# houzhijian/CONE

Measured on AMD Instinct MI355X. Metric: windows/sec + queries/sec, Ego4D-NLQ win_len=90 d=256 top-k=20, higher is better.
Workload: dtype f32

## Files before the change

### cone_amd/csrc/attention.hip

```cpp
#include "common.h"

#ifndef CONE_ATTN_NT
#define CONE_ATTN_NT 0
#endif

namespace cone {

constexpr float kQScale = 0.17677669529663687f;
constexpr float kQScaleLog2 = 0.17677669529663687f * 1.4426950408889634f;


typedef float f32x4m __attribute__((ext_vector_type(4)));
typedef float f32x2m __attribute__((ext_vector_type(2)));

__device__ __forceinline__ float lane_xor(float v, int lane, int mask) {
    return __int_as_float(__builtin_amdgcn_ds_bpermute((lane ^ mask) << 2, __float_as_int(v)));
}

template <int NKT>
__device__ __forceinline__ float attn_softmax(f32x4m (&sc)[NKT], int L, int lane, int lg) {
    const int lim = L - lg;
    float m = -INFINITY;
#pragma unroll
    for (int kt = 0; kt < NKT; ++kt) {
        if (16 * (kt + 1) > L) {
#pragma unroll
            for (int r = 0; r < 4; ++r) sc[kt][r] = (16 * kt + 4 * r < lim) ? sc[kt][r] : -INFINITY;
        }
#pragma unroll
        for (int r = 0; r < 4; ++r) m = fmaxf(m, sc[kt][r]);
    }
    m = fmaxf(m, lane_xor(m, lane, 16));
    m = fmaxf(m, lane_xor(m, lane, 32));
    const f32x2m m2 = {m, m};
    f32x2m l2 = {0.f, 0.f};
#pragma unroll
    for (int kt = 0; kt < NKT; ++kt) {
        f32x2m a = sc[kt].xy - m2, b = sc[kt].zw - m2;
        a.x = __builtin_amdgcn_exp2f(a.x); a.y = __builtin_amdgcn_exp2f(a.y);
        b.x = __builtin_amdgcn_exp2f(b.x); b.y = __builtin_amdgcn_exp2f(b.y);
        sc[kt].xy = a; sc[kt].zw = b;
        l2 += a;
        l2 += b;
    }
    float l = l2.x + l2.y;
    l += lane_xor(l, lane, 16);
    l += lane_xor(l, lane, 32);
    return 1.0f / l;
}

__device__ __forceinline__ void attn_normalise(f32x4m& o0, f32x4m& o1, float inv, int lane, int lg) {
#pragma unroll
    for (int r = 0; r < 4; ++r) {
        const float s = __int_as_float(__builtin_amdgcn_ds_bpermute(((lane & 48) + 4 * lg + r) << 2, __float_as_int(inv)));
        o0[r] *= s;
        o1[r] *= s;
    }
}

template <int NKT, int MODE_>
__global__ __launch_bounds__(64 * NKT, (NKT > 12 ? 4 : 6)) void enc_attn16_kernel(AttnSrc a, float* __restrict__ OUT,
                                                                 const int* __restrict__ off) {
    constexpr int MODE = MODE_ & 3;
    constexpr bool TXT = (MODE_ & 4) != 0;
    constexpr int KP = 16 * NKT, LDK = KP + 2, LDV = 36, NT = 64 * NKT;
    constexpr bool DYN = NKT > 12;
    __shared__ float KsT_s[DYN ? 4 : 32 * LDK];
    __shared__ __attribute__((aligned(16))) float Vs_s[DYN ? 4 : KP * LDV];
    extern __shared__ __attribute__((aligned(16))) float attn_dyn[];
    float* const KsT = DYN ? attn_dyn : KsT_s;
    float* const Vs = DYN ? attn_dyn + 32 * LDK : Vs_s;
    const int b = blockIdx.y, head = blockIdx.x;
    const int t0 = off[b];
    const int L = off[b + 1] - t0;
    if (L <= 0) return;
    const int tid = threadIdx.x, lane = tid & 63;
    const int wave = __builtin_amdgcn_readfirstlane(tid >> 6);
    const int li = lane & 15, lg = lane >> 4;
    const unsigned hc = head * 32;
    int lv = 0;
    const float *qb = nullptr, *kb = nullptr, *vb = nullptr, *tb = nullptr, *pb = nullptr;
    unsigned sq = 768, sk = 768, sv = 768;
    int pbase = 0;
    if (MODE != ATTN_PACKED) {
        lv = a.vlen[b];
        pbase = lv * (lv - 1) / 2;
        pb = a.pos_qk + hc;
    }
    if (MODE == ATTN_GATHER) {
        qb = a.qkv_vid + (size_t)a.vrow0[b] * 768 + hc;
        tb = a.qkv_txt + ((ptrdiff_t)a.trow0[b] - lv) * 768 + hc;
    } else {
        sq = a.ldq; sk = a.ldk; sv = a.ldv;
        qb = a.Q + (size_t)t0 * sq + hc; kb = a.K + (size_t)t0 * sk + hc; vb = a.V + (size_t)t0 * sv + hc;
    }
    const int zrow = a.pos_zero_row;
    const float* tpb = nullptr;
    if (TXT) tpb = a.txt_pos_qk + ((ptrdiff_t)a.trow0[b] - lv) * 512 + hc;
    auto prow = [&](int row) -> const float* {
        if (TXT && row >= lv) return tpb + (unsigned)row * 512u;
        return pb + (unsigned)(row < lv ? pbase + row : zrow) * 512u;
    };

    const int q0 = wave * 16;
    const int kr = tid >> 3;
    const unsigned c4 = (tid & 7) * 4;
    f32x4m qx[2], qt[2], kv[2], vv[2], kt_[2];
    {
        const int qrow = min(q0 + li, L - 1);
        const float* qp;
        if (MODE == ATTN_GATHER) qp = (qrow < lv ? qb : tb) + (unsigned)qrow * 768u + 8u * lg;
        else qp = qb + (unsigned)qrow * sq + 8u * lg;
        qx[0] = *reinterpret_cast<const f32x4m*>(qp);
        qx[1] = *reinterpret_cast<const f32x4m*>(qp + 4);
        if (MODE != ATTN_PACKED) {
            const float* pr = prow(qrow) + 8u * lg;
            qt[0] = *reinterpret_cast<const f32x4m*>(pr);
            qt[1] = *reinterpret_cast<const f32x4m*>(pr + 4);
        }
    }
#pragma unroll
    for (int it = 0; it < 2; ++it) {
        const int row = min(kr + it * (NT / 8), L - 1);
        if (MODE == ATTN_GATHER) {
            const float* rp = (row < lv ? qb : tb) + (unsigned)row * 768u + c4;
            kv[it] = *reinterpret_cast<const f32x4m*>(rp + 256);
            vv[it] = *reinterpret_cast<const f32x4m*>(rp + 512);
        } else {
#if CONE_ATTN_NT
            kv[it] = __builtin_nontemporal_load(reinterpret_cast<const f32x4m*>(kb + (unsigned)row * sk + c4));
            vv[it] = __builtin_nontemporal_load(reinterpret_cast<const f32x4m*>(vb + (unsigned)row * sv + c4));
#else
            kv[it] = *reinterpret_cast<const f32x4m*>(kb + (unsigned)row * sk + c4);
            vv[it] = *reinterpret_cast<const f32x4m*>(vb + (unsigned)row * sv + c4);
#endif
        }
        if (MODE != ATTN_PACKED)
            kt_[it] = *reinterpret_cast<const f32x4m*>(prow(row) + 256u + c4);
    }
    float qv[8];
    {
        f32x4m x0 = qx[0], x1 = qx[1];
        if (MODE != ATTN_PACKED) { x0 += qt[0]; x1 += qt[1]; }
        x0 *= kQScaleLog2; x1 *= kQScaleLog2;
#pragma unroll
        for (int j = 0; j < 4; ++j) { qv[j] = x0[j]; qv[4 + j] = x1[j]; }
    }
#pragma unroll
    for (int it = 0; it < 2; ++it) {
        const int key = kr + it * (NT / 8);
        f32x4m k4 = kv[it];
        if (MODE != ATTN_PACKED) k4 += kt_[it];
        const int pos = (key & ~15) + 4 * (key & 3) + ((key >> 2) & 3);
        float* kd = KsT + c4 * LDK + pos;
        kd[0] = k4[0]; kd[LDK] = k4[1]; kd[2 * LDK] = k4[2]; kd[3 * LDK] = k4[3];
        *reinterpret_cast<f32x4m*>(Vs + pos * LDV + c4) = vv[it];
    }
    __syncthreads();
    if (q0 >= L) return;

    f32x4m sc[NKT];
#pragma unroll
    for (int kt = 0; kt < NKT; ++kt) sc[kt] = f32x4m{0.f, 0.f, 0.f, 0.f};
#pragma unroll
    for (int st = 0; st < 8; ++st) {
        const float* kp = KsT + (8 * lg + st) * LDK + li;
#pragma unroll
        for (int kt = 0; kt < NKT; ++kt)
            sc[kt] = __builtin_amdgcn_mfma_f32_16x16x4f32(kp[kt * 16], qv[st], sc[kt], 0, 0, 0);
    }
    const float inv = attn_softmax<NKT>(sc, L, lane, lg);
    f32x4m o0 = {0.f, 0.f, 0.f, 0.f}, o1 = o0;
#pragma unroll
    for (int kt = 0; kt < NKT; ++kt) {
        const float* vp = Vs + (kt * 16 + 4 * lg) * LDV + li;
#pragma unroll
        for (int r = 0; r < 4; ++r) {
            if (kt < NKT - 2 || 16 * kt + 4 * r < L) {
                o0 = __builtin_amdgcn_mfma_f32_16x16x4f32(sc[kt][r], vp[r * LDV], o0, 0, 0, 0);
                o1 = __builtin_amdgcn_mfma_f32_16x16x4f32(sc[kt][r], vp[r * LDV + 16], o1, 0, 0, 0);
            }
        }
    }
    attn_normalise(o0, o1, inv, lane, lg);
    float* ob = OUT + (size_t)t0 * 256 + hc;
    const int qr0 = q0 + 4 * lg;
    const unsigned oo = (unsigned)qr0 * 256u + li;
#pragma unroll
    for (int r = 0; r < 4; ++r) {
        if (qr0 + r < L) {
            ob[oo + 256u * r] = o0[r];
            ob[oo + 256u * r + 16u] = o1[r];
        }
    }
}

template <int NKT, int MODE>
__global__ __launch_bounds__(256, 2) void enc_attn_wave_kernel(AttnSrc a, float* __restrict__ OUT,
                                                               const int* __restrict__ off) {
    const int b = blockIdx.y;
    const int lane = threadIdx.x & 63;
    const int head = blockIdx.x * 4 + __builtin_amdgcn_readfirstlane(threadIdx.x >> 6);
    const int t0 = off[b];
    const int L = off[b + 1] - t0;
    if (L <= 0) return;
    const int li = lane & 15, lg = lane >> 4;
    const unsigned hc = head * 32;
    int lv = 0, pbase = 0;
    const float *qb = nullptr, *kb = nullptr, *vb = nullptr, *tb = nullptr, *pb = nullptr;
    unsigned sq = 768, sk = 768, sv = 768;
    if (MODE != ATTN_PACKED) { lv = a.vlen[b]; pbase = lv * (lv - 1) / 2; pb = a.pos_qk + hc; }
    if (MODE == ATTN_GATHER) {
        qb = a.qkv_vid + (size_t)a.vrow0[b] * 768 + hc;
        tb = a.qkv_txt + ((ptrdiff_t)a.trow0[b] - lv) * 768 + hc;
    } else {
        sq = a.ldq; sk = a.ldk; sv = a.ldv;
        qb = a.Q + (size_t)t0 * sq + hc; kb = a.K + (size_t)t0 * sk + hc; vb = a.V + (size_t)t0 * sv + hc;
    }
    const int zrow = a.pos_zero_row;
    auto qptr = [&](int tok) { return MODE == ATTN_GATHER ? (tok < lv ? qb : tb) + (unsigned)tok * 768u : qb + (unsigned)tok * sq; };
    auto kptr = [&](int tok) { return MODE == ATTN_GATHER ? (tok < lv ? qb : tb) + (unsigned)tok * 768u + 256 : kb + (unsigned)tok * sk; };
    auto vptr = [&](int tok) { return MODE == ATTN_GATHER ? (tok < lv ? qb : tb) + (unsigned)tok * 768u + 512 : vb + (unsigned)tok * sv; };
    auto pptr = [&](int tok) { return pb + (unsigned)(tok < lv ? pbase + tok : zrow) * 512u; };
    f32x4m qx[2], qt[2];
    auto load_q = [&](int q0) {
        const int qrow = min(q0 + li, L - 1);
        const float* qp = qptr(qrow) + 8 * lg;
        qx[0] = *reinterpret_cast<const f32x4m*>(qp);
        qx[1] = *reinterpret_cast<const f32x4m*>(qp + 4);
        if (MODE != ATTN_PACKED) {
            const float* ap = pptr(qrow) + 8 * lg;
            qt[0] = *reinterpret_cast<const f32x4m*>(ap);
            qt[1] = *reinterpret_cast<const f32x4m*>(ap + 4);
        }
    };
    load_q(0);
    float kreg[NKT][8];
#pragma unroll
    for (int kt = 0; kt < NKT; ++kt) {
        const int key = min(16 * kt + 4 * (li & 3) + (li >> 2), L - 1);
        const float* kp_ = kptr(key) + 8 * lg;
#pragma unroll
        for (int u = 0; u < 2; ++u) {
            f32x4m k4 = *reinterpret_cast<const f32x4m*>(kp_ + 4 * u);
            if (MODE != ATTN_PACKED) k4 += *reinterpret_cast<const f32x4m*>(pptr(key) + 256 + 8 * lg + 4 * u);
#pragma unroll
            for (int j = 0; j < 4; ++j) kreg[kt][4 * u + j] = k4[j];
        }
    }
    float vreg[NKT][4][2];
#pragma unroll
    for (int kt = 0; kt < NKT; ++kt)
#pragma unroll
        for (int r = 0; r < 4; ++r) {
            const float* vp_ = vptr(min(16 * kt + 4 * r + lg, L - 1));
            vreg[kt][r][0] = vp_[li];
            vreg[kt][r][1] = vp_[16 + li];
        }
    for (int q0 = 0; q0 < L; q0 += 16) {
        float qv[8];
        {
            f32x4m x0 = qx[0], x1 = qx[1];
            if (MODE != ATTN_PACKED) { x0 += qt[0]; x1 += qt[1]; }
            x0 *= kQScaleLog2; x1 *= kQScaleLog2;
#pragma unroll
            for (int j = 0; j < 4; ++j) { qv[j] = x0[j]; qv[4 + j] = x1[j]; }
        }
        load_q(q0 + 16 < L ? q0 + 16 : q0);
        f32x4m sc[NKT];
#pragma unroll
        for (int kt = 0; kt < NKT; ++kt) sc[kt] = f32x4m{0.f, 0.f, 0.f, 0.f};
#pragma unroll
        for (int st = 0; st < 8; ++st)
#pragma unroll
            for (int kt = 0; kt < NKT; ++kt)
                sc[kt] = __builtin_amdgcn_mfma_f32_16x16x4f32(kreg[kt][st], qv[st], sc[kt], 0, 0, 0);
        const float inv = attn_softmax<NKT>(sc, L, lane, lg);
        f32x4m o0 = {0.f, 0.f, 0.f, 0.f}, o1 = o0;
#pragma unroll
        for (int kt = 0; kt < NKT; ++kt)
#pragma unroll
            for (int r = 0; r < 4; ++r) {
                o0 = __builtin_amdgcn_mfma_f32_16x16x4f32(sc[kt][r], vreg[kt][r][0], o0, 0, 0, 0);
                o1 = __builtin_amdgcn_mfma_f32_16x16x4f32(sc[kt][r], vreg[kt][r][1], o1, 0, 0, 0);
            }
        attn_normalise(o0, o1, inv, lane, lg);
#pragma unroll
        for (int r = 0; r < 4; ++r) {
            const int qrow = q0 + 4 * lg + r;
            if (qrow < L) {
                float* dst = OUT + (size_t)(t0 + qrow) * 256 + hc + li;
                dst[0] = o0[r];
                dst[16] = o1[r];
            }
        }
    }
}

template <int MODE>
static int launch_enc_attn_t(const AttnSrc& a, float* OUT, const int* off, int B, int Lmax, hipStream_t s) {
    const int nkt = max(6, (Lmax + 15) / 16);
    if (a.form == 2 && nkt <= 9 && !(MODE & 4)) {
        dim3 wgrid(2, B);
#define CONE_ATTNW(N) case N: hipLaunchKernelGGL((enc_attn_wave_kernel<N, (MODE & 3)>), wgrid, dim3(256), 0, s, a, OUT, off); break;
        switch (nkt) { CONE_ATTNW(6) CONE_ATTNW(7) CONE_ATTNW(8) CONE_ATTNW(9) }
#undef CONE_ATTNW
        CONE_LAUNCH_CHECK();
        return 0;
    }
    dim3 grid(8, B);
#define CONE_ATTN16(N) case N: hipLaunchKernelGGL((enc_attn16_kernel<N, MODE>), grid, dim3(64 * N), 0, s, a, OUT, off); break;
#define CONE_ATTN16D(N)                                                                                                     \
    case N: {                                                                                                               \
        constexpr int bytes = (32 * (16 * N + 2) + 16 * N * 36) * 4;                                                        \
        static DeviceOnce once;                                                                                             \
        CONE_CHECK_HIP(device_once(once, [] {                                                                               \
            return hipFuncSetAttribute((const void*)enc_attn16_kernel<N, MODE>, hipFuncAttributeMaxDynamicSharedMemorySize, bytes); \
        }));                                                                                                                \
        hipLaunchKernelGGL((enc_attn16_kernel<N, MODE>), grid, dim3(64 * N), bytes, s, a, OUT, off);                        \
        break;                                                                                                              \
    }
    switch (nkt) {
        CONE_ATTN16(6)
        CONE_ATTN16(7) CONE_ATTN16(8) CONE_ATTN16(9) CONE_ATTN16(10) CONE_ATTN16(11) CONE_ATTN16(12)
        CONE_ATTN16D(13) CONE_ATTN16D(14) CONE_ATTN16D(15) CONE_ATTN16D(16)
    }
#undef CONE_ATTN16
#undef CONE_ATTN16D
    CONE_LAUNCH_CHECK();
    return 0;
}

int launch_enc_attn(int mode, const AttnSrc& a, float* OUT, const int* off, int B, int Lmax, hipStream_t s) {
    CONE_REQUIRE(Lmax >= 1 && Lmax <= 256, "enc attention: window length %d not in [1,256]", Lmax);
    if (B <= 0) return 0;
    ProfScope ps(PK_ENC_ATTN, B, Lmax, mode, nullptr, s);
    switch (mode) {
        case ATTN_PACKED:
            CONE_REQUIRE(a.Q && a.K && a.V, "enc attention: packed mode needs Q, K, V");
            return launch_enc_attn_t<ATTN_PACKED>(a, OUT, off, B, Lmax, s);
        case ATTN_GATHER:
            CONE_REQUIRE(a.qkv_vid && a.qkv_txt && a.pos_qk && a.vrow0 && a.vlen && a.trow0 && a.pos_zero_row >= 0,
                         "enc attention: gather mode needs the layer-0 caches");
            if (a.txt_pos_qk) return launch_enc_attn_t<ATTN_GATHER | 4>(a, OUT, off, B, Lmax, s);
            return launch_enc_attn_t<ATTN_GATHER>(a, OUT, off, B, Lmax, s);
        case ATTN_POSADD:
            CONE_REQUIRE(a.Q && a.K && a.V && a.pos_qk && a.vlen && a.pos_zero_row >= 0,
                         "enc attention: pos-add mode needs Q, K, V, pos_qk, vlen");
            if (a.txt_pos_qk) {
                CONE_REQUIRE(a.trow0, "enc attention: text position rows need trow0");
                return launch_enc_attn_t<ATTN_POSADD | 4>(a, OUT, off, B, Lmax, s);
            }
            return launch_enc_attn_t<ATTN_POSADD>(a, OUT, off, B, Lmax, s);
    }
    set_error("enc attention: unknown mode %d", mode);
    return CONE_E_INVALID;
}

constexpr int kSmallMaxKeys = 192;
template <int MQ>
__global__ __launch_bounds__(64) void small_attn_kernel(const float* __restrict__ Q, int ldq,
                                                        const float* __restrict__ K, int ldk,
                                                        const float* __restrict__ V, int ldv,
                                                        float* __restrict__ OUT, int ldo,
                                                        const int* __restrict__ off, int nq) {
    __shared__ float qs[MQ][32];
    __shared__ float ps[MQ][kSmallMaxKeys];
    const int b = blockIdx.x, head = blockIdx.y, lane = threadIdx.x;
    const int k0 = off ? off[b] : b * nq;
    const int L = off ? off[b + 1] - k0 : nq;
    for (int i = lane; i < nq * 8; i += 64) {
        const int qi = i >> 3, c = i & 7;
        const float4 x = *reinterpret_cast<const float4*>(Q + (size_t)(b * nq + qi) * ldq + head * 32 + c * 4);
        qs[qi][c * 4] = x.x * kQScale; qs[qi][c * 4 + 1] = x.y * kQScale;
        qs[qi][c * 4 + 2] = x.z * kQScale; qs[qi][c * 4 + 3] = x.w * kQScale;
    }
    __syncthreads();
    float sc[3][MQ];
#pragma unroll
    for (int jj = 0; jj < 3; ++jj) {
        const int j = lane + 64 * jj;
#pragma unroll
        for (int qi = 0; qi < MQ; ++qi) sc[jj][qi] = -INFINITY;
        if (j < L) {
            float kv[32];
            const float* kp = K + (size_t)(k0 + j) * ldk + head * 32;
#pragma unroll
            for (int u = 0; u < 8; ++u) {
                const float4 x = reinterpret_cast<const float4*>(kp)[u];
                kv[4 * u] = x.x; kv[4 * u + 1] = x.y; kv[4 * u + 2] = x.z; kv[4 * u + 3] = x.w;
            }
#pragma unroll
            for (int qi = 0; qi < MQ; ++qi)
                if (qi < nq) {
                    float a = 0.f;
#pragma unroll
                    for (int d = 0; d < 32; ++d) a = fmaf(qs[qi][d], kv[d], a);
                    sc[jj][qi] = a;
                }
        }
    }
#pragma unroll
    for (int qi = 0; qi < MQ; ++qi)
        if (qi < nq) {
            const float m = wave_max(fmaxf(fmaxf(sc[0][qi], sc[1][qi]), sc[2][qi]));
            float e[3], l = 0.f;
#pragma unroll
            for (int jj = 0; jj < 3; ++jj) {
                e[jj] = (lane + 64 * jj < L) ? expf(sc[jj][qi] - m) : 0.f;
                l += e[jj];
            }
            const float inv = 1.0f / wave_sum(l);
#pragma unroll
            for (int jj = 0; jj < 3; ++jj)
                if (lane + 64 * jj < L) ps[qi][lane + 64 * jj] = e[jj] * inv;
        }
    __syncthreads();
    const int d = lane & 31, h = lane >> 5;
    float o[MQ];
#pragma unroll
    for (int qi = 0; qi < MQ; ++qi) o[qi] = 0.f;
    for (int j = h; j < L; j += 2) {
        const float v = V[(size_t)(k0 + j) * ldv + head * 32 + d];
#pragma unroll
        for (int qi = 0; qi < MQ; ++qi)
            if (qi < nq) o[qi] = fmaf(ps[qi][j], v, o[qi]);
    }
#pragma unroll
    for (int qi = 0; qi < MQ; ++qi)
        if (qi < nq) {
            const float t = o[qi] + __shfl_xor(o[qi], 32, 64);
            if (h == 0) OUT[(size_t)(b * nq + qi) * ldo + head * 32 + d] = t;
        }
}

template <int NQ>
__global__ __launch_bounds__(256) void dec_self_attn_kernel(const float* __restrict__ Q, int ldq, const float* __restrict__ K,
                                                            int ldk, const float* __restrict__ V, int ldv,
                                                            float* __restrict__ OUT, int ldo, int B) {
    const int b = blockIdx.x * 4 + (threadIdx.x >> 6);
    if (b >= B) return;
    const int lane = threadIdx.x & 63;
    float4 q[NQ], k[NQ], v[NQ];
#pragma unroll
    for (int i = 0; i < NQ; ++i) {
        const size_t row = (size_t)b * NQ + i;
        q[i] = reinterpret_cast<const float4*>(Q + row * ldq)[lane];
        k[i] = reinterpret_cast<const float4*>(K + row * ldk)[lane];
        v[i] = reinterpret_cast<const float4*>(V + row * ldv)[lane];
    }
#pragma unroll
    for (int i = 0; i < NQ; ++i) {
        float sc[NQ];
        float m = -INFINITY;
#pragma unroll
        for (int j = 0; j < NQ; ++j) {
            float d = ((q[i].x * kQScale) * k[j].x + (q[i].y * kQScale) * k[j].y) + ((q[i].z * kQScale) * k[j].z + (q[i].w * kQScale) * k[j].w);
            d += __shfl_xor(d, 1, 64);
            d += __shfl_xor(d, 2, 64);
            d += __shfl_xor(d, 4, 64);
            sc[j] = d;
            m = fmaxf(m, d);
        }
        float l = 0.f;
#pragma unroll
        for (int j = 0; j < NQ; ++j) { sc[j] = expf(sc[j] - m); l += sc[j]; }
        const float inv = 1.0f / l;
        float4 o = make_float4(0.f, 0.f, 0.f, 0.f);
#pragma unroll
        for (int j = 0; j < NQ; ++j) {
            const float p = sc[j] * inv;
            o.x = fmaf(p, v[j].x, o.x); o.y = fmaf(p, v[j].y, o.y); o.z = fmaf(p, v[j].z, o.z); o.w = fmaf(p, v[j].w, o.w);
        }
        reinterpret_cast<float4*>(OUT + ((size_t)b * NQ + i) * ldo)[lane] = o;
    }
}

int launch_small_attn(const float* Q, int ldq, const float* K, int ldk, const float* V, int ldv, float* OUT,
                      int ldo, const int* off, int B, int nq, int Lmax, hipStream_t s) {
    CONE_REQUIRE(nq >= 1 && nq <= 16, "decoder attention: num_queries=%d not in [1,16]", nq);
    CONE_REQUIRE(Lmax <= kSmallMaxKeys, "decoder attention: %d keys > %d", Lmax, kSmallMaxKeys);
    if (B <= 0) return 0;
    if (!off && (ldq | ldk | ldv | ldo) % 4 == 0) {
#define CONE_DSA(N)                                                                                                            \
        if (nq == N) {                                                                                                         \
            hipLaunchKernelGGL(dec_self_attn_kernel<N>, dim3((B + 3) / 4), dim3(256), 0, s, Q, ldq, K, ldk, V, ldv, OUT, ldo, B); \
            CONE_LAUNCH_CHECK();                                                                                               \
            return 0;                                                                                                          \
        }
        CONE_DSA(5) CONE_DSA(3) CONE_DSA(8) CONE_DSA(10)
#undef CONE_DSA
    }
    if (nq <= 8)
        hipLaunchKernelGGL(small_attn_kernel<8>, dim3(B, 8), dim3(64), 0, s, Q, ldq, K, ldk, V, ldv, OUT, ldo, off, nq);
    else
        hipLaunchKernelGGL(small_attn_kernel<16>, dim3(B, 8), dim3(64), 0, s, Q, ldq, K, ldk, V, ldv, OUT, ldo, off, nq);
    CONE_LAUNCH_CHECK();
    return 0;
}

}
```

Before: 379,500.

## Split encoder attention into full and short-window paths, byte-offset addressing

Adds separate compile-time paths for windows that fill the last two key tiles and for shorter windows. The short path skips QK and PV matrix-core work on the two trailing key tiles and avoids exponentials on fully masked tiles. It also rewrites global addressing to precomputed byte offsets, stores unguarded output rows when a wave's 16 queries are all valid, and adds asm barriers to shape instruction scheduling in the exp/sum loop. The cost is code duplication and higher register pressure, and a new stride cap is checked at launch.

Result: no change. 383,100 (median of 6 runs) (+0.9%).

```diff
diff --git a/cone_amd/csrc/attention.hip b/cone_amd/csrc/attention.hip
--- a/cone_amd/csrc/attention.hip
+++ b/cone_amd/csrc/attention.hip
@@ -17,31 +17,78 @@
     return __int_as_float(__builtin_amdgcn_ds_bpermute((lane ^ mask) << 2, __float_as_int(v)));
 }
 
-template <int NKT>
-__device__ __forceinline__ float attn_softmax(f32x4m (&sc)[NKT], int L, int lane, int lg) {
+#ifndef CONE_ATTN_PK
+#define CONE_ATTN_PK 0
+#endif
+template <bool FIRST>
+__device__ __forceinline__ void attn_exp_tile(f32x4m& s, float m, f32x2m& l2) {
+#if CONE_ATTN_PK
+    const f32x2m m2 = {m, m};
+    f32x2m a = s.xy - m2, b = s.zw - m2;
+    asm("" : "+v"(a));
+    asm("" : "+v"(b));
+    a.x = __builtin_amdgcn_exp2f(a.x); a.y = __builtin_amdgcn_exp2f(a.y);
+    b.x = __builtin_amdgcn_exp2f(b.x); b.y = __builtin_amdgcn_exp2f(b.y);
+    asm("" : "+v"(a));
+    asm("" : "+v"(b));
+    s.xy = a; s.zw = b;
+    if (FIRST) l2 = a; else l2 += a;
+    l2 += b;
+    asm("" : "+v"(l2));
+#else
+    float e[4];
+#pragma unroll
+    for (int r = 0; r < 4; ++r) {
+        e[r] = s[r] - m;
+        asm("" : "+v"(e[r]));
+        e[r] = __builtin_amdgcn_exp2f(e[r]);
+        s[r] = e[r];
+    }
+    float lx = l2.x, ly = l2.y;
+    if (FIRST) { lx = e[0]; ly = e[1]; }
+    else {
+        lx += e[0];
+        asm("" : "+v"(lx));
+        ly += e[1];
+        asm("" : "+v"(ly));
+    }
+    lx += e[2];
+    asm("" : "+v"(lx));
+    ly += e[3];
+    asm("" : "+v"(ly));
+    l2.x = lx; l2.y = ly;
+#endif
+}
+
+__device__ __forceinline__ void attn_mask_tile(f32x4m& s, int kt, int lim) {
+#pragma unroll
+    for (int r = 0; r < 4; ++r) s[r] = (16 * kt + 4 * r < lim) ? s[r] : -INFINITY;
+}
+
+template <int NKT, bool FULL>
+__device__ __forceinline__ float attn_softmax_path(f32x4m (&sc)[NKT], int L, int lane, int lg) {
     const int lim = L - lg;
+    if (!FULL) __builtin_assume(L <= 16 * (NKT - 2));
     float m = -INFINITY;
 #pragma unroll
     for (int kt = 0; kt < NKT; ++kt) {
-        if (16 * (kt + 1) > L) {
-#pragma unroll
-            for (int r = 0; r < 4; ++r) sc[kt][r] = (16 * kt + 4 * r < lim) ? sc[kt][r] : -INFINITY;
+        if (FULL) {
+            if (kt == NKT - 1 || (kt == NKT - 2 && 16 * (kt + 1) > L)) attn_mask_tile(sc[kt], kt, lim);
+        } else {
+            if (16 * kt >= L) continue;
+            if (16 * (kt + 1) > L) attn_mask_tile(sc[kt], kt, lim);
         }
 #pragma unroll
         for (int r = 0; r < 4; ++r) m = fmaxf(m, sc[kt][r]);
     }
     m = fmaxf(m, lane_xor(m, lane, 16));
     m = fmaxf(m, lane_xor(m, lane, 32));
-    const f32x2m m2 = {m, m};
     f32x2m l2 = {0.f, 0.f};
-#pragma unroll
-    for (int kt = 0; kt < NKT; ++kt) {
-        f32x2m a = sc[kt].xy - m2, b = sc[kt].zw - m2;
-        a.x = __builtin_amdgcn_exp2f(a.x); a.y = __builtin_amdgcn_exp2f(a.y);
-        b.x = __builtin_amdgcn_exp2f(b.x); b.y = __builtin_amdgcn_exp2f(b.y);
-        sc[kt].xy = a; sc[kt].zw = b;
-        l2 += a;
-        l2 += b;
+    attn_exp_tile<true>(sc[0], m, l2);
+#pragma unroll
+    for (int kt = 1; kt < NKT; ++kt) {
+        if (!FULL && 16 * kt >= L) sc[kt] = f32x4m{0.f, 0.f, 0.f, 0.f};
+        else attn_exp_tile<false>(sc[kt], m, l2);
     }
     float l = l2.x + l2.y;
     l += lane_xor(l, lane, 16);
@@ -49,6 +96,12 @@
     return 1.0f / l;
 }
 
+template <int NKT>
+__device__ __forceinline__ float attn_softmax(f32x4m (&sc)[NKT], int L, int lane, int lg) {
+    if (L > 16 * (NKT - 2)) return attn_softmax_path<NKT, true>(sc, L, lane, lg);
+    return attn_softmax_path<NKT, false>(sc, L, lane, lg);
+}
+
 __device__ __forceinline__ void attn_normalise(f32x4m& o0, f32x4m& o1, float inv, int lane, int lg) {
 #pragma unroll
     for (int r = 0; r < 4; ++r) {
@@ -56,6 +109,55 @@
         o0[r] *= s;
         o1[r] *= s;
     }
+}
+
+__device__ __forceinline__ f32x4m ldg4(const float* base, unsigned byte_off) {
+    return *reinterpret_cast<const f32x4m*>(reinterpret_cast<const char*>(base) + byte_off);
+}
+__device__ __forceinline__ void stg(float* base, unsigned byte_off, float v) {
+    *reinterpret_cast<float*>(reinterpret_cast<char*>(base) + byte_off) = v;
+}
+
+template <int NKT, bool FULL>
+__device__ __forceinline__ float attn_core16(const float* KsT, const float* Vs, const float (&qv)[8], int L, int lane, int li,
+                                             int lg, f32x4m& o0, f32x4m& o1) {
+    constexpr int LDK = 16 * NKT + 2, LDV = 36;
+    f32x4m sc[NKT];
+#pragma unroll
+    for (int kt = 0; kt < NKT; ++kt) sc[kt] = f32x4m{0.f, 0.f, 0.f, 0.f};
+    if (FULL) {
+#pragma unroll
+        for (int st = 0; st < 8; ++st) {
+            const float* kp = KsT + (8 * lg + st) * LDK + li;
+#pragma unroll
+            for (int kt = 0; kt < NKT; ++kt)
+                sc[kt] = __builtin_amdgcn_mfma_f32_16x16x4f32(kp[kt * 16], qv[st], sc[kt], 0, 0, 0);
+        }
+    } else {
+#pragma unroll
+        for (int kt = 0; kt < NKT - 2; ++kt) {
+            if (16 * kt < L) {
+#pragma unroll
+                for (int st = 0; st < 8; ++st)
+                    sc[kt] = __builtin_amdgcn_mfma_f32_16x16x4f32(KsT[(8 * lg + st) * LDK + li + kt * 16], qv[st], sc[kt], 0, 0, 0);
+            }
+        }
+    }
+    const float inv = attn_softmax_path<NKT, FULL>(sc, L, lane, lg);
+    o0 = f32x4m{0.f, 0.f, 0.f, 0.f};
+    o1 = o0;
+#pragma unroll
+    for (int kt = 0; kt < (FULL ? NKT : NKT - 2); ++kt) {
+        const float* vp = Vs + (kt * 16 + 4 * lg) * LDV + li;
+#pragma unroll
+        for (int r = 0; r < 4; ++r) {
+            if ((FULL && kt < NKT - 2) || 16 * kt + 4 * r < L) {
+                o0 = __builtin_amdgcn_mfma_f32_16x16x4f32(sc[kt][r], vp[r * LDV], o0, 0, 0, 0);
+                o1 = __builtin_amdgcn_mfma_f32_16x16x4f32(sc[kt][r], vp[r * LDV + 16], o1, 0, 0, 0);
+            }
+        }
+    }
+    return inv;
 }
 
 template <int NKT, int MODE_>
@@ -80,7 +182,7 @@
     const unsigned hc = head * 32;
     int lv = 0;
     const float *qb = nullptr, *kb = nullptr, *vb = nullptr, *tb = nullptr, *pb = nullptr;
-    unsigned sq = 768, sk = 768, sv = 768;
+    unsigned sq = 3072, sk = 3072, sv = 3072;
     int pbase = 0;
     if (MODE != ATTN_PACKED) {
         lv = a.vlen[b];
@@ -91,15 +193,15 @@
         qb = a.qkv_vid + (size_t)a.vrow0[b] * 768 + hc;
         tb = a.qkv_txt + ((ptrdiff_t)a.trow0[b] - lv) * 768 + hc;
     } else {
-        sq = a.ldq; sk = a.ldk; sv = a.ldv;
-        qb = a.Q + (size_t)t0 * sq + hc; kb = a.K + (size_t)t0 * sk + hc; vb = a.V + (size_t)t0 * sv + hc;
+        sq = 4u * a.ldq; sk = 4u * a.ldk; sv = 4u * a.ldv;
+        qb = a.Q + (size_t)t0 * a.ldq + hc; kb = a.K + (size_t)t0 * a.ldk + hc; vb = a.V + (size_t)t0 * a.ldv + hc;
     }
     const int zrow = a.pos_zero_row;
     const float* tpb = nullptr;
     if (TXT) tpb = a.txt_pos_qk + ((ptrdiff_t)a.trow0[b] - lv) * 512 + hc;
-    auto prow = [&](int row) -> const float* {
-        if (TXT && row >= lv) return tpb + (unsigned)row * 512u;
-        return pb + (unsigned)(row < lv ? pbase + row : zrow) * 512u;
+    auto ldpos = [&](int row, unsigned col) -> f32x4m {
+        if (TXT) return ldg4(row >= lv ? tpb : pb, (unsigned)(row >= lv ? row : pbase + row) * 2048u + col);
+        return ldg4(pb, (unsigned)(row < lv ? pbase + row : zrow) * 2048u + col);
     };
 
     const int q0 = wave * 16;
@@ -108,35 +210,39 @@
     f32x4m qx[2], qt[2], kv[2], vv[2], kt_[2];
     {
         const int qrow = min(q0 + li, L - 1);
-        const float* qp;
-        if (MODE == ATTN_GATHER) qp = (qrow < lv ? qb : tb) + (unsigned)qrow * 768u + 8u * lg;
-        else qp = qb + (unsigned)qrow * sq + 8u * lg;
-        qx[0] = *reinterpret_cast<const f32x4m*>(qp);
-        qx[1] = *reinterpret_cast<const f32x4m*>(qp + 4);
+        if (MODE == ATTN_GATHER) {
+            const float* src = qrow < lv ? qb : tb;
+            const unsigned o = (unsigned)qrow * 3072u + 32u * lg;
+            qx[0] = ldg4(src, o);
+            qx[1] = ldg4(src, o + 16u);
+        } else {
+            const unsigned o = (unsigned)qrow * sq + 32u * lg;
+            qx[0] = ldg4(qb, o);
+            qx[1] = ldg4(qb, o + 16u);
+        }
         if (MODE != ATTN_PACKED) {
-            const float* pr = prow(qrow) + 8u * lg;
-            qt[0] = *reinterpret_cast<const f32x4m*>(pr);
-            qt[1] = *reinterpret_cast<const f32x4m*>(pr + 4);
+            qt[0] = ldpos(qrow, 32u * lg);
+            qt[1] = ldpos(qrow, 32u * lg + 16u);
         }
     }
 #pragma unroll
     for (int it = 0; it < 2; ++it) {
         const int row = min(kr + it * (NT / 8), L - 1);
         if (MODE == ATTN_GATHER) {
-            const float* rp = (row < lv ? qb : tb) + (unsigned)row * 768u + c4;
-            kv[it] = *reinterpret_cast<const f32x4m*>(rp + 256);
-            vv[it] = *reinterpret_cast<const f32x4m*>(rp + 512);
+            const float* src = row < lv ? qb : tb;
+            const unsigned o = (unsigned)row * 3072u + 4u * c4;
+            kv[it] = ldg4(src, o + 1024u);
+            vv[it] = ldg4(src, o + 2048u);
         } else {
 #if CONE_ATTN_NT
-            kv[it] = __builtin_nontemporal_load(reinterpret_cast<const f32x4m*>(kb + (unsigned)row * sk + c4));
-            vv[it] = __builtin_nontemporal_load(reinterpret_cast<const f32x4m*>(vb + (unsigned)row * sv + c4));
+            kv[it] = __builtin_nontemporal_load(reinterpret_cast<const f32x4m*>(reinterpret_cast<const char*>(kb) + ((unsigned)row * sk + 4u * c4)));
+            vv[it] = __builtin_nontemporal_load(reinterpret_cast<const f32x4m*>(reinterpret_cast<const char*>(vb) + ((unsigned)row * sv + 4u * c4)));
 #else
-            kv[it] = *reinterpret_cast<const f32x4m*>(kb + (unsigned)row * sk + c4);
-            vv[it] = *reinterpret_cast<const f32x4m*>(vb + (unsigned)row * sv + c4);
+            kv[it] = ldg4(kb, (unsigned)row * sk + 4u * c4);
+            vv[it] = ldg4(vb, (unsigned)row * sv + 4u * c4);
 #endif
         }
-        if (MODE != ATTN_PACKED)
-            kt_[it] = *reinterpret_cast<const f32x4m*>(prow(row) + 256u + c4);
+        if (MODE != ATTN_PACKED) kt_[it] = ldpos(row, 1024u + 4u * c4);
     }
     float qv[8];
     {
@@ -159,38 +265,27 @@
     __syncthreads();
     if (q0 >= L) return;
 
-    f32x4m sc[NKT];
-#pragma unroll
-    for (int kt = 0; kt < NKT; ++kt) sc[kt] = f32x4m{0.f, 0.f, 0.f, 0.f};
-#pragma unroll
-    for (int st = 0; st < 8; ++st) {
-        const float* kp = KsT + (8 * lg + st) * LDK + li;
-#pragma unroll
-        for (int kt = 0; kt < NKT; ++kt)
-            sc[kt] = __builtin_amdgcn_mfma_f32_16x16x4f32(kp[kt * 16], qv[st], sc[kt], 0, 0, 0);
-    }
-    const float inv = attn_softmax<NKT>(sc, L, lane, lg);
-    f32x4m o0 = {0.f, 0.f, 0.f, 0.f}, o1 = o0;
-#pragma unroll
-    for (int kt = 0; kt < NKT; ++kt) {
-        const float* vp = Vs + (kt * 16 + 4 * lg) * LDV + li;
-#pragma unroll
-        for (int r = 0; r < 4; ++r) {
-            if (kt < NKT - 2 || 16 * kt + 4 * r < L) {
-                o0 = __builtin_amdgcn_mfma_f32_16x16x4f32(sc[kt][r], vp[r * LDV], o0, 0, 0, 0);
-                o1 = __builtin_amdgcn_mfma_f32_16x16x4f32(sc[kt][r], vp[r * LDV + 16], o1, 0, 0, 0);
-            }
-        }
-    }
+    f32x4m o0, o1;
+    float inv;
+    if (L > 16 * (NKT - 2)) inv = attn_core16<NKT, true>(KsT, Vs, qv, L, lane, li, lg, o0, o1);
+    else inv = attn_core16<NKT, false>(KsT, Vs, qv, L, lane, li, lg, o0, o1);
     attn_normalise(o0, o1, inv, lane, lg);
     float* ob = OUT + (size_t)t0 * 256 + hc;
     const int qr0 = q0 + 4 * lg;
-    const unsigned oo = (unsigned)qr0 * 256u + li;
-#pragma unroll
-    for (int r = 0; r < 4; ++r) {
-        if (qr0 + r < L) {
-            ob[oo + 256u * r] = o0[r];
-            ob[oo + 256u * r + 16u] = o1[r];
+    const unsigned oo = (unsigned)qr0 * 1024u + 4u * li;
+    if (q0 + 16 <= L) {
+#pragma unroll
+        for (int r = 0; r < 4; ++r) {
+            stg(ob, oo + 1024u * r, o0[r]);
+            stg(ob, oo + 1024u * r + 64u, o1[r]);
+        }
+    } else {
+#pragma unroll
+        for (int r = 0; r < 4; ++r) {
+            if (qr0 + r < L) {
+                stg(ob, oo + 1024u * r, o0[r]);
+                stg(ob, oo + 1024u * r + 64u, o1[r]);
+            }
         }
     }
 }
@@ -331,6 +426,8 @@
     return 0;
 }
 
+constexpr int kEncAttnMaxLd = 1 << 22;
+
 int launch_enc_attn(int mode, const AttnSrc& a, float* OUT, const int* off, int B, int Lmax, hipStream_t s) {
     CONE_REQUIRE(Lmax >= 1 && Lmax <= 256, "enc attention: window length %d not in [1,256]", Lmax);
     if (B <= 0) return 0;
@@ -338,6 +435,7 @@
     switch (mode) {
         case ATTN_PACKED:
             CONE_REQUIRE(a.Q && a.K && a.V, "enc attention: packed mode needs Q, K, V");
+            CONE_REQUIRE(max(a.ldq, max(a.ldk, a.ldv)) <= kEncAttnMaxLd, "enc attention: row stride above %d floats", kEncAttnMaxLd);
             return launch_enc_attn_t<ATTN_PACKED>(a, OUT, off, B, Lmax, s);
         case ATTN_GATHER:
             CONE_REQUIRE(a.qkv_vid && a.qkv_txt && a.pos_qk && a.vrow0 && a.vlen && a.trow0 && a.pos_zero_row >= 0,
@@ -347,6 +445,7 @@
         case ATTN_POSADD:
             CONE_REQUIRE(a.Q && a.K && a.V && a.pos_qk && a.vlen && a.pos_zero_row >= 0,
                          "enc attention: pos-add mode needs Q, K, V, pos_qk, vlen");
+            CONE_REQUIRE(max(a.ldq, max(a.ldk, a.ldv)) <= kEncAttnMaxLd, "enc attention: row stride above %d floats", kEncAttnMaxLd);
             if (a.txt_pos_qk) {
                 CONE_REQUIRE(a.trow0, "enc attention: text position rows need trow0");
                 return launch_enc_attn_t<ATTN_POSADD | 4>(a, OUT, off, B, Lmax, s);
```
